# burn-research/OpenMEASURE

Measured on AMD Instinct MI355X. Metric: SPR fit+reconstruct throughput (GB/s snapshot matrix), higher is better.
Workload: dtype f64

## Files before the change

openmeasure_amd/csrc/common.hpp:

```cpp
#pragma once
#include <hip/hip_runtime.h>
#include <stdint.h>
#include <stdio.h>

#include "spr_hip.h"

typedef double f64x4 __attribute__((ext_vector_type(4)));
typedef double f64x2 __attribute__((ext_vector_type(2)));

void spr_set_error(const char *fmt, ...);

#define SPR_REQUIRE(cond, code, ...)      \
  do {                                    \
    if (!(cond)) {                        \
      spr_set_error(__VA_ARGS__);         \
      return (code);                      \
    }                                     \
  } while (0)

#define SPR_HIP_TRY(expr)                                                          \
  do {                                                                             \
    hipError_t e__ = (expr);                                                       \
    if (e__ != hipSuccess) {                                                       \
      spr_set_error("%s failed: %s (%s:%d)", #expr, hipGetErrorString(e__),       \
// ... 42 lines not shown
__host__ __device__ inline int seg_first_feature(const SegPlan &p) { return (int)(p.row0 / p.n_points); }
__host__ __device__ inline int seg_last_feature(const SegPlan &p) {
  int64_t f = (p.row0 + p.n_rows - 1) / p.n_points;
  if (f > p.n_features - 1) f = p.n_features - 1;
  return (int)f;
}

inline int seg_total_wgs(const SegPlan &p) {
  int tot = 0;
  for (int f = seg_first_feature(p); f <= seg_last_feature(p); ++f) {
    int64_t lo, hi;
    seg_range(p, f, lo, hi);
    tot += seg_wgs(p, hi - lo);
  }
  return tot;
}

__device__ inline bool seg_locate(const SegPlan &p, int b, int &f, int &wl, int &wpf, int &base,
                                  int64_t &lo, int64_t &hi) {
  int acc = 0;
  int f1 = seg_last_feature(p);
  for (int ff = seg_first_feature(p); ff <= f1; ++ff) {
    seg_range(p, ff, lo, hi);
    int w = seg_wgs(p, hi - lo);
    if (b < acc + w) {
      f = ff; wl = b - acc; wpf = w; base = acc;
      return true;
    }
    acc += w;
  }
  return false;
}

template <int CTRL>
__device__ inline double dpp_f64(double v) {
  union { double d; int i[2]; } a, b;
  a.d = v;
  b.i[0] = __builtin_amdgcn_update_dpp(0, a.i[0], CTRL, 0xF, 0xF, true);
  b.i[1] = __builtin_amdgcn_update_dpp(0, a.i[1], CTRL, 0xF, 0xF, true);
  return b.d;
}

template <int WIDTH>
__device__ inline double group_sum_t(double v) {
  if (WIDTH >= 2) v += dpp_f64<0xB1>(v);
  if (WIDTH >= 4) v += dpp_f64<0x4E>(v);
  if (WIDTH >= 8) v += dpp_f64<0x141>(v);
  if (WIDTH >= 16) v += dpp_f64<0x140>(v);
  if (WIDTH >= 32) v += __shfl_xor(v, 16, 64);
  if (WIDTH >= 64) v += __shfl_xor(v, 32, 64);
  return v;
}

__device__ inline double group_sum(double v, int width) {
  for (int o = width >> 1; o > 0; o >>= 1) v += __shfl_xor(v, o, 64);
  return v;
}

constexpr int spr_pow2_divisor_le64(int n) {
  int p = 1;
  while (p < 64 && n % (2 * p) == 0) p *= 2;
  return p;
}

inline int spr_round_mt(int m) {
  static const int sup[] = {1, 2, 3, 4, 6, 8, 12, 16};
  int need = (m + 15) / 16;
  for (int s : sup)
    if (s >= need) return s;
  return -1;
}
```

openmeasure_amd/csrc/qr_pivot.hip:

```cpp
#include <stdlib.h>

#include <type_traits>

#include "rowtile.hpp"

namespace {

constexpr int QR_THREADS = 256;
#ifndef QR_EPOCH_DEEP
#define QR_EPOCH_DEEP 0
#endif
#ifndef QR_ABLATE
#define QR_ABLATE 0
#endif
#ifndef QR_TOPT_N
#define QR_TOPT_N 16
#endif
constexpr int QR_TOPT = QR_TOPT_N;
constexpr int QR_MAX_BLOCKS = 1024;
constexpr int QR_BATCH = 16;

struct Best {
  double v1; int64_t i1; double v2;
  __device__ inline void init() { v1 = -2.0; i1 = INT64_MAX; v2 = -2.0; }
// ... 60 lines not shown
    bv = -3.0; bi = INT64_MAX; bp = -1;
    for (int e = first + lane; e < first + count; e += 64) {
      const double v = sval[e]; const long long i = sidx[e];
      if (v > bv || (v == bv && i < bi)) { bv = v; bi = i; bp = e; }
    }
    for (int o = 32; o > 0; o >>= 1) {
      const double ov = __shfl_xor(bv, o, 64);
      const long long oi = __shfl_xor(bi, o, 64);
      const int op = __shfl_xor(bp, o, 64);
      if (ov > bv || (ov == bv && oi < bi)) { bv = ov; bi = oi; bp = op; }
    }
  }
  template <int SPW>
  __device__ inline void block_merge(double *sval, long long *sidx, double *out, bool owner, int slot) {
    constexpr int NWV = QR_THREADS / 64;
    __shared__ double wv[NWV * QR_TOPT];
    __shared__ long long wi[NWV * QR_TOPT];
    const int lane = threadIdx.x & 63, wave = threadIdx.x >> 6;
    if (owner) {
#pragma unroll
      for (int k = 0; k < QR_TOPT; ++k) {
        sval[(wave * SPW + slot) * QR_TOPT + k] = tv[k];
        sidx[(wave * SPW + slot) * QR_TOPT + k] = ti[k] >= 0 ? (long long)ti[k] + base : -1;
      }
    }
    __syncthreads();
    for (int round = 0; round < QR_TOPT; ++round) {
      double bv; long long bi; int bp;
      argmax_round(sval, sidx, wave * SPW * QR_TOPT, SPW * QR_TOPT, lane, bv, bi, bp);
      if (lane == 0) {
        wv[wave * QR_TOPT + round] = bv;
        wi[wave * QR_TOPT + round] = bi;
        if (bp >= 0) sval[bp] = -3.0;
      }
      __builtin_amdgcn_wave_barrier();
    }
    __syncthreads();
    if (wave == 0) {
      for (int round = 0; round < QR_TOPT; ++round) {
        double bv; long long bi; int bp;
        argmax_round(wv, wi, 0, NWV * QR_TOPT, lane, bv, bi, bp);
        if (lane == 0) {
          out[2 * round] = bv > -2.5 ? bv : -2.0;
          out[2 * round + 1] = (double)(bv > -2.5 ? bi : -1);
          if (bp >= 0) wv[bp] = -3.0;
        }
        __builtin_amdgcn_wave_barrier();
      }
    }
  }
};
using TopList = TopListT<long long>;

template <bool INIT>
struct RowOwner {
  int off, q;
  bool own;
  __device__ inline RowOwner(int lane) {
    const int g = lane >> 4, c = lane & 15;
    if (INIT) { off = c; q = c >> 2; own = (c & 3) == g; }
    else { off = g + 4 * (c & 3); q = c & 3; own = c < 4; }
  }
  __device__ inline int slot(int lane) const { return INIT ? ((lane >> 4) * 4 + ((lane & 15) >> 2)) : ((lane >> 4) * 4 + (lane & 3)); }
  __device__ inline double pick(double v0, double v1, double v2, double v3) const {
    return q == 0 ? v0 : q == 1 ? v1 : q == 2 ? v2 : v3;
  }
};
constexpr int QR_SPW = 16;

template <int MTR, int VEC, typename TU, bool INIT>
__global__ __launch_bounds__(QR_THREADS) void qr_refresh_mfma_kernel(
    const TU *__restrict__ Ur, int64_t n_rows, int r, int64_t ldu, int64_t row0,
    const double *__restrict__ Q, int nq, double *__restrict__ nrm, double *__restrict__ tops) {
  constexpr int NW = QR_THREADS / 64, R = 64;
  constexpr int MPAD = 16 * MTR, MP = MPAD + 2, KSTEPS = MPAD / 4;
  using RT = RowTile<MTR, R, MP, NW, 16, TU>;
  constexpr int SPW = QR_SPW;
  constexpr int PANELS = 2 * R * MP, MERGE = 2 * (QR_THREADS / 64) * SPW * QR_TOPT;
  __shared__ double smem[PANELS > MERGE ? PANELS : MERGE];
  double *const lds0 = smem, *const lds1 = smem + R * MP;
  double *const sval = smem;
  long long *const sidx = reinterpret_cast<long long *>(smem + (QR_THREADS / 64) * SPW * QR_TOPT);
  const int lane = threadIdx.x & 63;
  const int wave = __builtin_amdgcn_readfirstlane(threadIdx.x >> 6);

  double bfrag[KSTEPS];
#pragma unroll
  for (int ks = 0; ks < KSTEPS; ++ks) {
    const int k = 4 * ks + (lane >> 4), j = lane & 15;
    bfrag[ks] = (!INIT && j < nq && k < r) ? Q[(int64_t)j * r + k] : 0.0;
  }
  TopList top;
  top.init();
  const RowOwner<INIT> who(lane);
  RT tile;
  const int64_t npanels = (n_rows + R - 1) / R;
  int64_t c = blockIdx.x;
  if (c < npanels) {
    tile.template load<VEC>(Ur, ldu, r, c * R, n_rows, wave, lane);
    tile.raw_store(lds0, r, c * R, n_rows, wave, lane);
    int64_t cn = c + gridDim.x;
    int64_t nrow0 = (cn < npanels) ? cn * R : n_rows;
    tile.template load<VEC>(Ur, ldu, r, nrow0, n_rows, wave, lane);
    int buf = 0;
    const int afrag = (lane & 15) * MP + (lane >> 4);
    auto old_of = [&](int64_t row0p) {
      const int64_t rr = row0p + wave * 16 + who.off;
      return (INIT || QR_ABLATE >= 2) ? 0.0 : nrm[rr < n_rows ? rr : n_rows - 1];
    };
    double old = old_of(c * R), old_n = old_of(nrow0);
    while (c < npanels) {
      const double *cur = buf ? lds1 : lds0;
      double *nxt = buf ? lds0 : lds1;
      const int64_t c2 = cn + gridDim.x;
      const int64_t n2row0 = (c2 < npanels) ? c2 * R : n_rows;
      __syncthreads();
      const int64_t orow = c * R + wave * 16 + who.off;
      const bool mine = who.own && orow < n_rows;
      const double old_n2 = old_of(n2row0);
      const double *p = cur + wave * 16 * MP + afrag;
      f64x4 acc = {0.0, 0.0, 0.0, 0.0};
#pragma unroll
      for (int ks = 0; ks < KSTEPS; ++ks) {
        const double a = p[4 * ks];
        acc = __builtin_amdgcn_mfma_f64_16x16x4f64(a, INIT ? a : bfrag[ks], acc, 0, 0, 0);
        if (ks == 0) {
#pragma unroll
          for (int it = 0; it < RT::IT; ++it) {
            tile.raw_store_pass(it, nxt, r, nrow0, n_rows, wave, lane);
            tile.template load_pass<VEC>(it, Ur, ldu, r, n2row0, n_rows, wave, lane);
          }
        }
      }
      double v;
      if (INIT) {
        v = who.pick(acc.x, acc.y, acc.z, acc.w);
      } else {
        const double d2 = who.pick(group_sum_t<16>(acc.x * acc.x), group_sum_t<16>(acc.y * acc.y),
                                   group_sum_t<16>(acc.z * acc.z), group_sum_t<16>(acc.w * acc.w));
        v = old - d2;
        v = v < 0.0 ? 0.0 : v;
        v = old < 0.0 ? -1.0 : v;
      }
      if (QR_ABLATE >= 2) asm volatile("" ::"v"(v));
      if (QR_ABLATE < 2 && mine) nrm[orow] = v;
      if (QR_ABLATE < 1) top.insert(v, row0 + orow, mine);
      old = old_n;
      old_n = old_n2;
      buf ^= 1;
      c = cn;
      cn = c2;
      nrow0 = n2row0;
    }
  }
  __syncthreads();
  top.template block_merge<SPW>(sval, sidx, tops + (int64_t)blockIdx.x * QR_TOPT * 2, who.own, who.slot(lane));
}

template <int NG, typename TU, bool INIT>
__global__ __launch_bounds__(QR_THREADS) void qr_refresh_direct_kernel(
    const TU *__restrict__ Ur, int64_t n_rows, int r, int64_t ldu, int64_t row0,
    const double *__restrict__ Q, int nq, double *__restrict__ nrm, double *__restrict__ tops) {
  constexpr int R = 64;
  constexpr int SPW = QR_SPW;
  __shared__ double smem[2 * (QR_THREADS / 64) * SPW * QR_TOPT];
  double *const sval = smem;
  long long *const sidx = reinterpret_cast<long long *>(smem + (QR_THREADS / 64) * SPW * QR_TOPT);
  const int lane = threadIdx.x & 63;
  const int wave = __builtin_amdgcn_readfirstlane(threadIdx.x >> 6);
  const int li = lane & 15, kk = lane >> 4;
  using P4 = typename std::conditional<std::is_same<TU, float>::value, float4, double4>::type;

  double bfrag[4 * NG];
#pragma unroll
  for (int g = 0; g < NG; ++g)
#pragma unroll
    for (int t = 0; t < 4; ++t)
      bfrag[4 * g + t] = (!INIT && li < nq) ? Q[(int64_t)li * r + 16 * g + 4 * kk + t] : 0.0;
  TopList top;
  top.init();
  const RowOwner<INIT> who(lane);
  const int64_t npanels = (n_rows + R - 1) / R;
  auto load_block = [&](int64_t c, P4 (&dst)[NG]) {
    int64_t row = c * R + wave * 16 + li;
    row = row < n_rows ? row : n_rows - 1;
    const TU *rp = Ur + row * ldu + 4 * kk;
#pragma unroll
    for (int g = 0; g < NG; ++g) dst[g] = *reinterpret_cast<const P4 *>(rp + 16 * g);
  };
  auto old_of = [&](int64_t cc) {
    const int64_t rr = cc * R + wave * 16 + who.off;
    return INIT ? 0.0 : nrm[rr < n_rows ? rr : n_rows - 1];
  };
  int64_t c = blockIdx.x;
  P4 cur[NG], nxt[NG];
  double old = 0.0;
  if (c < npanels) { load_block(c, cur); old = old_of(c); }
  while (c < npanels) {
    const int64_t cn = c + gridDim.x;
    load_block(cn < npanels ? cn : c, nxt);
    const double old_n = old_of(cn < npanels ? cn : c);
    const int64_t orow = c * R + wave * 16 + who.off;
    const bool mine = who.own && orow < n_rows;
    f64x4 acc = {0.0, 0.0, 0.0, 0.0};
#pragma unroll
    for (int g = 0; g < NG; ++g) {
      const double a4[4] = {(double)cur[g].x, (double)cur[g].y, (double)cur[g].z, (double)cur[g].w};
#pragma unroll
      for (int t = 0; t < 4; ++t)
        acc = __builtin_amdgcn_mfma_f64_16x16x4f64(a4[t], INIT ? a4[t] : bfrag[4 * g + t], acc, 0, 0, 0);
    }
    double v;
    if (INIT) {
      v = who.pick(acc.x, acc.y, acc.z, acc.w);
    } else {
      const double d2 = who.pick(group_sum_t<16>(acc.x * acc.x), group_sum_t<16>(acc.y * acc.y),
                                 group_sum_t<16>(acc.z * acc.z), group_sum_t<16>(acc.w * acc.w));
      v = old - d2;
      v = v < 0.0 ? 0.0 : v;
      v = old < 0.0 ? -1.0 : v;
    }
    if (mine) nrm[orow] = v;
    top.insert(v, row0 + orow, mine);
#pragma unroll
    for (int g = 0; g < NG; ++g) cur[g] = nxt[g];
    old = old_n;
    c = cn;
  }
  top.template block_merge<SPW>(sval, sidx, tops + (int64_t)blockIdx.x * QR_TOPT * 2, who.own, who.slot(lane));
}

template <int NGMAX, int VEC, typename TU, bool INIT>
__global__ __launch_bounds__(QR_THREADS) void qr_refresh_wide_kernel(
    const TU *__restrict__ Ur, int64_t n_rows, int r, int64_t ldu, int64_t row0,
    const double *__restrict__ Q, int nq, double *__restrict__ nrm, double *__restrict__ tops) {
  constexpr int R = 64, SG = 8;
  constexpr int SPW = QR_SPW;
  __shared__ double smem[2 * (QR_THREADS / 64) * SPW * QR_TOPT];
  __shared__ double Ql[INIT ? 16 : NGMAX * 256];
  double *const sval = smem;
  long long *const sidx = reinterpret_cast<long long *>(smem + (QR_THREADS / 64) * SPW * QR_TOPT);
  const int lane = threadIdx.x & 63;
  const int wave = __builtin_amdgcn_readfirstlane(threadIdx.x >> 6);
  const int li = lane & 15, kk = lane >> 4;
  const int ng = (r + 15) / 16;
  using P4 = typename std::conditional<std::is_same<TU, float>::value, float4, double4>::type;

  if (!INIT) {
    for (int e = threadIdx.x; e < ng * 256; e += QR_THREADS) {
      const int j = e & 15, k4 = (e >> 4) & 3, t = (e >> 6) & 3, g = e >> 8;
      const int k = 16 * g + 4 * k4 + t;
      Ql[e] = (j < nq && k < r) ? Q[(int64_t)j * r + k] : 0.0;
    }
    __syncthreads();
  }
  TopList top;
  top.init();
  const RowOwner<INIT> who(lane);
  const int64_t npanels = (n_rows + R - 1) / R;
  auto load_batch = [&](const TU *rp, int g0, P4 (&dst)[SG]) {
#pragma unroll
    for (int u = 0; u < SG; ++u) {
      const int g = g0 + u < ng ? g0 + u : ng - 1;
      const int c0 = 16 * g + 4 * kk;
      if (VEC) {
        dst[u] = *reinterpret_cast<const P4 *>(rp + c0);
      } else {
        dst[u].x = c0 < r ? rp[c0] : (TU)0;         dst[u].y = c0 + 1 < r ? rp[c0 + 1] : (TU)0;
        dst[u].z = c0 + 2 < r ? rp[c0 + 2] : (TU)0; dst[u].w = c0 + 3 < r ? rp[c0 + 3] : (TU)0;
      }
    }
  };
  for (int64_t c = blockIdx.x; c < npanels; c += gridDim.x) {
    int64_t row = c * R + wave * 16 + li;
    row = row < n_rows ? row : n_rows - 1;
    const TU *rp = Ur + row * ldu;
    const int64_t orow = c * R + wave * 16 + who.off;
    const bool mine = who.own && orow < n_rows;
    const double old = INIT ? 0.0 : nrm[orow < n_rows ? orow : n_rows - 1];
    f64x4 acc = {0.0, 0.0, 0.0, 0.0};
    P4 cur[SG], nxt[SG];
    load_batch(rp, 0, cur);
    for (int g0 = 0; g0 < ng; g0 += SG) {
      load_batch(rp, g0 + SG, nxt);
#pragma unroll
      for (int u = 0; u < SG; ++u) {
        if (g0 + u < ng) {
          const double a4[4] = {(double)cur[u].x, (double)cur[u].y, (double)cur[u].z, (double)cur[u].w};
          const double *ql = Ql + (int64_t)(g0 + u) * 256 + kk * 16 + li;
#pragma unroll
          for (int t = 0; t < 4; ++t)
            acc = __builtin_amdgcn_mfma_f64_16x16x4f64(a4[t], INIT ? a4[t] : ql[64 * t], acc, 0, 0, 0);
        }
      }
#pragma unroll
      for (int u = 0; u < SG; ++u) cur[u] = nxt[u];
    }
    double v;
    if (INIT) {
      v = who.pick(acc.x, acc.y, acc.z, acc.w);
    } else {
      const double d2 = who.pick(group_sum_t<16>(acc.x * acc.x), group_sum_t<16>(acc.y * acc.y),
                                 group_sum_t<16>(acc.z * acc.z), group_sum_t<16>(acc.w * acc.w));
      v = old - d2;
      v = v < 0.0 ? 0.0 : v;
      v = old < 0.0 ? -1.0 : v;
    }
    if (mine) nrm[orow] = v;
    top.insert(v, row0 + orow, mine);
  }
  top.template block_merge<SPW>(sval, sidx, tops + (int64_t)blockIdx.x * QR_TOPT * 2, who.own, who.slot(lane));
}

__global__ __launch_bounds__(QR_THREADS) void qr_tops_from_norms_kernel(const double *__restrict__ nrm0, int64_t n_rows,
                                                                        int64_t row0, double *__restrict__ nrm,
                                                                        double *__restrict__ tops) {
  constexpr int R = 64, NWV = QR_THREADS / 64, SPW = 64;
  __shared__ double smem[2 * NWV * SPW * QR_TOPT];
  double *const sval = smem;
  long long *const sidx = reinterpret_cast<long long *>(smem + NWV * SPW * QR_TOPT);
  const int lane = threadIdx.x & 63, wave = threadIdx.x >> 6;
  TopList top;
  top.init();
  const int64_t npanels = (n_rows + R - 1) / R;
  const int64_t stride = (int64_t)gridDim.x * NWV;
  int64_t c = blockIdx.x + (int64_t)wave * gridDim.x;
  for (; (c + 3 * stride + 1) * R <= n_rows; c += 4 * stride) {
    double v[4];
#pragma unroll
    for (int u = 0; u < 4; ++u) v[u] = nrm0[(c + u * stride) * R + lane];
#pragma unroll
    for (int u = 0; u < 4; ++u) {
      const int64_t row = (c + u * stride) * R + lane;
      nrm[row] = v[u];
      top.insert(v[u], row0 + row, true);
    }
  }
  for (; c < npanels; c += stride) {
    const int64_t row = c * R + lane;
    const bool mine = row < n_rows;
    const double v = nrm0[mine ? row : n_rows - 1];
    if (mine) nrm[row] = v;
    top.insert(v, row0 + row, mine);
  }
  top.template block_merge<SPW>(sval, sidx, tops + (int64_t)blockIdx.x * QR_TOPT * 2, true, lane);
}

template <typename TU>
__global__ __launch_bounds__(QR_THREADS) void qr_gather_kernel(
    const double *__restrict__ tops, const TU *__restrict__ Ur, int r, int64_t ldu, int64_t row0,
    int64_t n_rows, int ldc, int64_t *__restrict__ cand_idx, double *__restrict__ cand_res,
    double *__restrict__ cand_U) {
  const int b = blockIdx.x;
  for (int e = threadIdx.x; e < QR_TOPT * ldc; e += QR_THREADS) {
    const int k = e / ldc, c = e - k * ldc;
    const double v = tops[((int64_t)b * QR_TOPT + k) * 2];
// ... 485 lines not shown
    else if (r <= 512) RWV(32);
    else RWV(64);
#undef RWV
#undef RW
    SPR_LAUNCH_CHECK();
    return SPR_OK;
  }
  const int mtr = spr_round_mt(r);
  const int lm = vec_ok ? ((r == 16 * mtr) ? 2 : 1) : 0;
  static const bool direct_on = [] { const char *e = getenv("SPR_QR_DIRECT"); return !(e && e[0] == '0'); }();
  const bool want_direct = INIT || std::is_same<TU, float>::value;
  if (direct_on && want_direct && r % 16 == 0 && (ldu * sizeof(TU)) % 16 == 0 &&
      (reinterpret_cast<uintptr_t>(Ur) & 15) == 0) {
#define RD(NGV) hipLaunchKernelGGL((qr_refresh_direct_kernel<NGV, TU, INIT>), dim3(grid), dim3(QR_THREADS), 0, st, Ur, n_rows, r, ldu, row0, Qj, nq, nrm, tops)
    switch (r / 16) {
      case 1: RD(1); break;
      case 2: RD(2); break;
      case 3: RD(3); break;
      case 4: RD(4); break;
      case 5: RD(5); break;
      case 6: RD(6); break;
      case 7: RD(7); break;
      default: RD(8); break;
    }
#undef RD
    SPR_LAUNCH_CHECK();
    return SPR_OK;
  }
#define RF(MTV, LM) hipLaunchKernelGGL((qr_refresh_mfma_kernel<MTV, LM, TU, INIT>), dim3(grid), dim3(QR_THREADS), 0, st, Ur, n_rows, r, ldu, row0, Qj, nq, nrm, tops)
#define RFV(MTV) do { if (lm == 2) RF(MTV, 2); else if (lm == 1) RF(MTV, 1); else RF(MTV, 0); } while (0)
  switch (mtr) {
    case 1: RFV(1); break;
    case 2: RFV(2); break;
    case 3: RFV(3); break;
    case 4: RFV(4); break;
    case 6: RFV(6); break;
    default: RFV(8); break;
  }
#undef RFV
#undef RF
  SPR_LAUNCH_CHECK();
  return SPR_OK;
}

int check_ur(const char *who, const void *Ur, int64_t n_rows, int32_t r, int64_t ldu) {
  SPR_REQUIRE(Ur != nullptr, SPR_E_INVALID, "%s: Ur is NULL", who);
  SPR_REQUIRE(n_rows > 0 && r > 0 && ldu >= r, SPR_E_INVALID, "%s: bad shape n_rows=%lld r=%d ldu=%lld", who,
              (long long)n_rows, r, (long long)ldu);
  SPR_REQUIRE(r <= SPR_MAX_R_WIDE, SPR_E_UNSUPPORTED, "%s: r=%d > %d not built", who, r, SPR_MAX_R_WIDE);
  return SPR_OK;
}

template <int NG, int NTT, typename P4>
__device__ inline void epoch_tiles_mfma(const P4 (&cur)[NG], const double *__restrict__ ql0, double (&q2)[4]) {
  f64x4 acc[NTT];
#pragma unroll
  for (int tl = 0; tl < NTT; ++tl) acc[tl] = f64x4{0.0, 0.0, 0.0, 0.0};
#pragma unroll
  for (int g = 0; g < NG; ++g) {
    const double a4[4] = {(double)cur[g].x, (double)cur[g].y, (double)cur[g].z, (double)cur[g].w};
#pragma unroll
    for (int t = 0; t < 4; ++t) {
#pragma unroll
      for (int tl = 0; tl < NTT; ++tl)
        acc[tl] = __builtin_amdgcn_mfma_f64_16x16x4f64(a4[t], ql0[tl * NG * 256 + (g * 4 + t) * 64], acc[tl], 0, 0, 0);
    }
  }
#pragma unroll
  for (int tl = 0; tl < NTT; ++tl) {
    q2[0] = fma(acc[tl].x, acc[tl].x, q2[0]); q2[1] = fma(acc[tl].y, acc[tl].y, q2[1]);
    q2[2] = fma(acc[tl].z, acc[tl].z, q2[2]); q2[3] = fma(acc[tl].w, acc[tl].w, q2[3]);
  }
}

template <int NG, int NT, typename TU, bool POOL, bool ILP = false>
__global__ __launch_bounds__(QR_THREADS, (NG <= 4 && !ILP ? 3 : 2)) void qr_epoch_sweep_kernel(
    const TU *__restrict__ Ur, int64_t n_rows, int r, int64_t ldu, int64_t row0, const double *__restrict__ Q, int nq,
    double *__restrict__ nrm_e, double *__restrict__ nrm, const int32_t *__restrict__ pool,
    const int32_t *__restrict__ pool_n_ptr, double *__restrict__ tops) {
  constexpr int R = 64, SPW = QR_SPW;
  __shared__ double smem[2 * (QR_THREADS / 64) * SPW * QR_TOPT];
  __shared__ double Ql[NT * NG * 256];
  double *const sval = smem;
  long long *const sidx = reinterpret_cast<long long *>(smem + (QR_THREADS / 64) * SPW * QR_TOPT);
  const int lane = threadIdx.x & 63;
  const int wave = __builtin_amdgcn_readfirstlane(threadIdx.x >> 6);
  const int li = lane & 15, kk = lane >> 4;
  using P4 = typename std::conditional<std::is_same<TU, float>::value, float4, double4>::type;
  const int nt = (nq + 15) / 16;
  for (int e = threadIdx.x; e < nt * NG * 256; e += QR_THREADS) {
    const int j = e & 15, k4 = (e >> 4) & 3, t = (e >> 6) & 3, g = (e >> 8) % NG, tile = (e >> 8) / NG;
    const int d = 16 * tile + j;
    Ql[e] = (d < nq) ? Q[(int64_t)d * r + 16 * g + 4 * k4 + t] : 0.0;
  }
  __syncthreads();
  TopListT<int> top;
  top.init();
  top.base = row0;
  const RowOwner<false> who(lane);
  const int64_t n_units = POOL ? (int64_t)*pool_n_ptr : n_rows;
  const int64_t npanels = (n_units + R - 1) / R;
  auto slot_row = [&](int64_t c) -> int64_t {
    const int64_t u = c * R + wave * 16 + li;
    if (u >= n_units) return -1;
    return POOL ? (int64_t)pool[u] : u;
  };
  auto load_block = [&](int64_t row, P4 (&dst)[NG]) {
    const TU *rp = Ur + (row >= 0 ? row : 0) * ldu + 4 * kk;
#pragma unroll
    for (int g = 0; g < NG; ++g) dst[g] = *reinterpret_cast<const P4 *>(rp + 16 * g);
  };
  auto own_row = [&](int64_t row) -> int64_t {
    const int lo = __shfl((int)(row & 0xffffffff), who.off, 64), hi = __shfl((int)(row >> 32), who.off, 64);
    return ((int64_t)hi << 32) | (uint32_t)lo;
  };
  constexpr int NBUF = (QR_EPOCH_DEEP && NG * sizeof(P4) / 4 <= 32 && NG <= 6) ? 3 : 2;
  P4 buf[NBUF][NG];
  double oldv[NBUF];
  int64_t orv[NBUF];
  auto fetch = [&](int64_t cc, P4 (&dst)[NG], double &old, int64_t &orow) {
    const int64_t row = cc < npanels ? slot_row(cc) : -1;
    load_block(row, dst);
    orow = own_row(row);
    old = nrm_e[orow >= 0 ? orow : 0];
  };
  auto process = [&](const P4 (&cur)[NG], double old, int64_t orow) {
    const bool mine = who.own && orow >= 0;
    double q2[4] = {0.0, 0.0, 0.0, 0.0};
    if (ILP) {
      const double *ql0 = Ql + kk * 16 + li;
      if (nt == 1) epoch_tiles_mfma<NG, 1, P4>(cur, ql0, q2);
      else if (nt == 2) epoch_tiles_mfma<NG, (NT >= 2 ? 2 : 1), P4>(cur, ql0, q2);
      else if (nt == 3) epoch_tiles_mfma<NG, (NT >= 3 ? 3 : 1), P4>(cur, ql0, q2);
      else epoch_tiles_mfma<NG, (NT >= 4 ? 4 : 1), P4>(cur, ql0, q2);
    } else
    for (int tile = 0; tile < nt; ++tile) {
      const double *ql = Ql + tile * NG * 256 + kk * 16 + li;
      f64x4 acc = {0.0, 0.0, 0.0, 0.0};
#pragma unroll
      for (int g = 0; g < NG; ++g) {
        const double a4[4] = {(double)cur[g].x, (double)cur[g].y, (double)cur[g].z, (double)cur[g].w};
#pragma unroll
        for (int t = 0; t < 4; ++t)
          acc = __builtin_amdgcn_mfma_f64_16x16x4f64(a4[t], ql[(g * 4 + t) * 64], acc, 0, 0, 0);
      }
      q2[0] = fma(acc.x, acc.x, q2[0]); q2[1] = fma(acc.y, acc.y, q2[1]);
      q2[2] = fma(acc.z, acc.z, q2[2]); q2[3] = fma(acc.w, acc.w, q2[3]);
    }
    const double d2 = who.pick(group_sum_t<16>(q2[0]), group_sum_t<16>(q2[1]), group_sum_t<16>(q2[2]), group_sum_t<16>(q2[3]));
    double v = old - d2;
    v = v < 0.0 ? 0.0 : v;
    v = old < 0.0 ? -1.0 : v;
    if (mine) {
      nrm[orow] = v;
      if (!POOL) nrm_e[orow] = v;
    }
    top.insert(v, (int)orow, mine);
  };
  int64_t c = blockIdx.x;
  const int64_t gs = gridDim.x;
#pragma unroll
  for (int u = 0; u < NBUF - 1; ++u) fetch(c + u * gs, buf[u], oldv[u], orv[u]);
  while (c < npanels) {
#pragma unroll
    for (int u = 0; u < NBUF; ++u) {
      if (c < npanels) {
        constexpr int NB1 = NBUF - 1;
        fetch(c + NB1 * gs, buf[(u + NB1) % NBUF], oldv[(u + NB1) % NBUF], orv[(u + NB1) % NBUF]);
        process(buf[u], oldv[u], orv[u]);
        c += gs;
      }
    }
  }
  top.template block_merge<SPW>(sval, sidx, tops + (int64_t)blockIdx.x * QR_TOPT * 2, who.own, who.slot(lane));
}

constexpr int PB_THREADS = 256;
constexpr int PB_MAX_BLOCKS = 2048;

__global__ __launch_bounds__(PB_THREADS) void qr_pool_count_kernel(const double *__restrict__ nrm_e, int64_t n_rows,
                                                                   int64_t chunk, double theta, int32_t *__restrict__ counts) {
  __shared__ int red[PB_THREADS / 64];
  const int64_t lo = (int64_t)blockIdx.x * chunk, hi = lo + chunk < n_rows ? lo + chunk : n_rows;
  int cnt = 0;
  for (int64_t i = lo + threadIdx.x; i < hi; i += PB_THREADS) cnt += nrm_e[i] > theta;
  for (int o = 32; o > 0; o >>= 1) cnt += __shfl_xor(cnt, o, 64);
  if ((threadIdx.x & 63) == 0) red[threadIdx.x >> 6] = cnt;
  __syncthreads();
  if (threadIdx.x == 0) {
    int t = 0;
    for (int w = 0; w < PB_THREADS / 64; ++w) t += red[w];
    counts[blockIdx.x] = t;
  }
}

__global__ __launch_bounds__(1024) void qr_pool_scan_kernel(int32_t *__restrict__ counts, int n_blocks, int64_t cap,
                                                            int32_t *__restrict__ pool_n) {
  constexpr int PER = (PB_MAX_BLOCKS + 1023) / 1024;
  __shared__ int wsum[16];
  const int t = threadIdx.x, lane = t & 63, wave = t >> 6;
  int v[PER], mine = 0;
#pragma unroll
  for (int i = 0; i < PER; ++i) {
    const int b = t * PER + i;
    v[i] = b < n_blocks ? counts[b] : 0;
    mine += v[i];
  }
  int incl = mine;
  for (int o = 1; o < 64; o <<= 1) {
    const int up = __shfl_up(incl, o, 64);
    if (lane >= o) incl += up;
  }
  if (lane == 63) wsum[wave] = incl;
  __syncthreads();
  int before = 0, total = 0;
  for (int w = 0; w < 16; ++w) { if (w < wave) before += wsum[w]; total += wsum[w]; }
  int run = before + incl - mine;
#pragma unroll
  for (int i = 0; i < PER; ++i) {
    const int b = t * PER + i;
    if (b < n_blocks) counts[b] = run;
    run += v[i];
  }
  if (t == 0) *pool_n = (int64_t)total <= cap ? total : -1;
}

__global__ __launch_bounds__(PB_THREADS) void qr_pool_fill_kernel(const double *__restrict__ nrm_e, int64_t n_rows,
// ... 260 lines not shown
                                  const int64_t *d_piv, int32_t nq, double d_min, void *stream) {
  SPR_REQUIRE(d_nrm && n_rows > 0 && row0 >= 0 && n_points > 0, SPR_E_INVALID, "spr_qr_exclude_f64: bad arguments");
  SPR_REQUIRE(nq >= 0 && nq <= QR_BATCH && (nq == 0 || (d_xyz && d_piv)), SPR_E_INVALID,
              "spr_qr_exclude_f64: nq=%d picks need xyz and piv (at most %d per call)", nq, QR_BATCH);
  SPR_REQUIRE(!d_xyz || (xyz_dim >= 1 && xyz_dim <= 3), SPR_E_INVALID, "spr_qr_exclude_f64: xyz needs 1..3 columns");
  if (!d_mask && nq == 0) return SPR_OK;
  int64_t blocks = (n_rows + QR_THREADS - 1) / QR_THREADS;
  if (blocks > 4096) blocks = 4096;
  hipLaunchKernelGGL(qr_exclude_kernel, dim3((int)blocks), dim3(QR_THREADS), 0, static_cast<hipStream_t>(stream), d_nrm,
                     n_rows, row0, n_points, d_mask, d_xyz, (int)xyz_dim, d_piv, (int)nq, d_min);
  SPR_LAUNCH_CHECK();
  return SPR_OK;
}

template <typename TU>
static int qr_refresh_entry(const char *who, const TU *d_Ur, int64_t n_rows, int32_t r, int64_t ldu, int64_t row0,
                            const double *d_Q, const int64_t *d_piv, int32_t j0, int32_t nq, double *d_nrm,
                            double *d_rec, double *d_tau, void *d_workspace, size_t workspace_bytes, void *stream) {
  int rc = check_ur(who, d_Ur, n_rows, r, ldu);
  if (rc != SPR_OK) return rc;
  SPR_REQUIRE(d_Q && d_piv && d_nrm && d_rec && d_tau && d_workspace, SPR_E_INVALID, "%s: NULL pointer", who);
  SPR_REQUIRE(j0 >= 0 && nq >= 1 && nq <= QR_BATCH && j0 + nq <= r, SPR_E_INVALID, "%s: bad j0=%d nq=%d", who, j0, nq);
  SPR_REQUIRE(workspace_bytes >= QrWs::bytes(r), SPR_E_WORKSPACE, "%s: workspace too small", who);
  hipStream_t st = static_cast<hipStream_t>(stream);
  const int grid = sweep_grid(n_rows);
  const int vec_ok = (r % 2 == 0) && (ldu % 2 == 0) && ((reinterpret_cast<uintptr_t>(d_Ur) & (2 * sizeof(TU) - 1)) == 0);
  QrWs w(d_workspace, r);
  hipLaunchKernelGGL(qr_mark_kernel, dim3(1), dim3(64), 0, st, d_piv + j0, (int)nq, row0, n_rows, d_nrm);
  SPR_LAUNCH_CHECK();
  rc = launch_refresh<TU, false>(grid, st, d_Ur, n_rows, (int)r, ldu, vec_ok, row0, d_Q + (int64_t)j0 * r, (int)nq, d_nrm, w.tops);
  if (rc != SPR_OK) return rc;
  return build_candidates<TU>(w, grid, d_Ur, n_rows, r, ldu, row0, d_rec, d_tau, st);
}

extern "C" int spr_qr_refresh_f64(const double *d_Ur, int64_t n_rows, int32_t r, int64_t ldu, int64_t row0,
                                  const double *d_Q, const int64_t *d_piv, int32_t j0, int32_t nq, double *d_nrm,
                                  double *d_rec, double *d_tau, void *d_workspace, size_t workspace_bytes,
                                  void *stream) {
  return qr_refresh_entry("spr_qr_refresh_f64", d_Ur, n_rows, r, ldu, row0, d_Q, d_piv, j0, nq, d_nrm, d_rec, d_tau,
                          d_workspace, workspace_bytes, stream);
}

extern "C" int spr_qr_refresh_u32(const float *d_Ur, int64_t n_rows, int32_t r, int64_t ldu, int64_t row0,
                                  const double *d_Q, const int64_t *d_piv, int32_t j0, int32_t nq, double *d_nrm,
                                  double *d_rec, double *d_tau, void *d_workspace, size_t workspace_bytes,
                                  void *stream) {
  return qr_refresh_entry("spr_qr_refresh_u32", d_Ur, n_rows, r, ldu, row0, d_Q, d_piv, j0, nq, d_nrm, d_rec, d_tau,
                          d_workspace, workspace_bytes, stream);
}

extern "C" int32_t spr_qr_epoch_supported(int32_t r, int64_t ldu, const void *d_Ur, int32_t u_is_f32, int64_t n_rows) {
  const size_t es = u_is_f32 ? sizeof(float) : sizeof(double);
  return r >= 16 && r <= SPR_MAX_R && r % 16 == 0 && (ldu * es) % 16 == 0 && (reinterpret_cast<uintptr_t>(d_Ur) & 15) == 0 &&
         n_rows > 0 && n_rows < INT32_MAX;
}

extern "C" int32_t spr_qr_epoch_max_directions(int32_t r) {
  const int ng = r / 16;
  return 16 * (ng < 4 ? ng : ng <= 6 ? 4 : 3);
}

extern "C" size_t spr_qr_pool_workspace(void) { return sizeof(int32_t) * (PB_MAX_BLOCKS + 4); }

extern "C" int spr_qr_pool_build(const double *d_nrm_e, int64_t n_rows, double theta, int32_t *d_pool, int64_t cap,
                                 int32_t *d_pool_n, void *d_workspace, size_t workspace_bytes, void *stream) {
  SPR_REQUIRE(d_nrm_e && d_pool && d_pool_n && d_workspace, SPR_E_INVALID, "spr_qr_pool_build: NULL pointer");
  SPR_REQUIRE(n_rows > 0 && n_rows < INT32_MAX && cap > 0, SPR_E_INVALID, "spr_qr_pool_build: bad shape");
  SPR_REQUIRE(workspace_bytes >= spr_qr_pool_workspace(), SPR_E_WORKSPACE, "spr_qr_pool_build: workspace too small");
  hipStream_t st = static_cast<hipStream_t>(stream);
  int64_t chunk = (n_rows + PB_MAX_BLOCKS - 1) / PB_MAX_BLOCKS;
  chunk = (chunk + PB_THREADS - 1) / PB_THREADS * PB_THREADS;
  const int blocks = (int)((n_rows + chunk - 1) / chunk);
  int32_t *counts = static_cast<int32_t *>(d_workspace);
  hipLaunchKernelGGL(qr_pool_count_kernel, dim3(blocks), dim3(PB_THREADS), 0, st, d_nrm_e, n_rows, chunk, theta, counts);
  SPR_LAUNCH_CHECK();
  hipLaunchKernelGGL(qr_pool_scan_kernel, dim3(1), dim3(1024), 0, st, counts, blocks, cap, d_pool_n);
  SPR_LAUNCH_CHECK();
  hipLaunchKernelGGL(qr_pool_fill_kernel, dim3(blocks), dim3(PB_THREADS), 0, st, d_nrm_e, n_rows, chunk, theta, counts,
                     d_pool_n, d_pool);
  SPR_LAUNCH_CHECK();
  return SPR_OK;
}

template <typename TU>
static int qr_epoch_entry(const char *who, const TU *d_Ur, int64_t n_rows, int32_t r, int64_t ldu, int64_t row0,
                          const double *d_Q, const int64_t *d_piv, int32_t j_e, int32_t j, int32_t j_mark,
                          double *d_nrm_e, double *d_nrm, const int32_t *d_pool, const int32_t *d_pool_n,
                          int64_t pool_n_host, double tau_floor, double *d_rec, double *d_tau, void *d_workspace,
                          size_t workspace_bytes, void *stream) {
  int rc = check_ur(who, d_Ur, n_rows, r, ldu);
  if (rc != SPR_OK) return rc;
  SPR_REQUIRE(d_Q && d_piv && d_nrm_e && d_nrm && d_rec && d_tau && d_workspace, SPR_E_INVALID, "%s: NULL pointer", who);
  SPR_REQUIRE(spr_qr_epoch_supported(r, ldu, d_Ur, std::is_same<TU, float>::value, n_rows), SPR_E_UNSUPPORTED,
              "%s: r=%d / alignment outside the epoch sweep's range (r a multiple of 16 up to %d, 16-byte rows)", who, r, SPR_MAX_R);
  SPR_REQUIRE(j_e >= 0 && j > j_e && j <= r && j - j_e <= spr_qr_epoch_max_directions(r) && j_mark >= 0 && j_mark <= j,
              SPR_E_INVALID, "%s: bad direction range [%d, %d) (at most %d per sweep), marks from %d", who, j_e, j,
              spr_qr_epoch_max_directions(r), j_mark);
  SPR_REQUIRE(!d_pool || (d_pool_n && pool_n_host >= 1 && pool_n_host <= n_rows), SPR_E_INVALID, "%s: bad pool", who);
  SPR_REQUIRE(workspace_bytes >= QrWs::bytes(r), SPR_E_WORKSPACE, "%s: workspace too small", who);
  hipStream_t st = static_cast<hipStream_t>(stream);
  QrWs w(d_workspace, r);
  for (int m0 = j_mark; m0 < j; m0 += 64) {
    const int nm = j - m0 < 64 ? j - m0 : 64;
    hipLaunchKernelGGL(qr_mark_kernel, dim3(1), dim3(64), 0, st, d_piv + m0, nm, row0, n_rows, d_nrm_e);
    hipLaunchKernelGGL(qr_mark_kernel, dim3(1), dim3(64), 0, st, d_piv + m0, nm, row0, n_rows, d_nrm);
  }
  SPR_LAUNCH_CHECK();
// ... 59 lines not shown
```

Baseline: 1104.

## Transpose MFMA operands so row norms reduce via permlane swaps and wave-level top list

Swaps the A/B operands of the f64 MFMA in the refresh and epoch kernels so each row's projection lands across lanes of a column. The squared norm then reduces with two permlane16/permlane32 swaps instead of four 16-wide DPP/shuffle reductions. The epoch kernel also replaces the per-slot top-K list with a wave-level sorted list kept one entry per lane, uses 32-bit row offsets for addressing, and shrinks shared memory. It adds a stride limit on the epoch path and relies on MI355X-specific permlane swap builtins.

```diff
diff --git a/openmeasure_amd/csrc/common.hpp b/openmeasure_amd/csrc/common.hpp
--- a/openmeasure_amd/csrc/common.hpp
+++ b/openmeasure_amd/csrc/common.hpp
@@ -118,6 +118,19 @@
   return v;
 }
 
+__device__ inline double rows_sum_f64(double v) {
+  union { double d; unsigned u[2]; } a, lo, hi;
+  a.d = v;
+  const auto s0 = __builtin_amdgcn_permlane16_swap(a.u[0], a.u[0], false, false);
+  const auto s1 = __builtin_amdgcn_permlane16_swap(a.u[1], a.u[1], false, false);
+  lo.u[0] = s0[0]; lo.u[1] = s1[0]; hi.u[0] = s0[1]; hi.u[1] = s1[1];
+  a.d = lo.d + hi.d;
+  const auto t0 = __builtin_amdgcn_permlane32_swap(a.u[0], a.u[0], false, false);
+  const auto t1 = __builtin_amdgcn_permlane32_swap(a.u[1], a.u[1], false, false);
+  lo.u[0] = t0[0]; lo.u[1] = t1[0]; hi.u[0] = t0[1]; hi.u[1] = t1[1];
+  return lo.d + hi.d;
+}
+
 __device__ inline double group_sum(double v, int width) {
   for (int o = width >> 1; o > 0; o >>= 1) v += __shfl_xor(v, o, 64);
   return v;
diff --git a/openmeasure_amd/csrc/qr_pivot.hip b/openmeasure_amd/csrc/qr_pivot.hip
--- a/openmeasure_amd/csrc/qr_pivot.hip
+++ b/openmeasure_amd/csrc/qr_pivot.hip
@@ -136,20 +136,79 @@
 };
 using TopList = TopListT<long long>;
 
+template <typename TI>
+struct WaveTopT {
+  static_assert(QR_TOPT <= 16 && sizeof(TI) == 4, "one list entry per lane of a 16-lane row; 32-bit row indices");
+  double tv, thr;
+  TI ti;
+  long long base = 0;
+  bool first;
+  __device__ inline void init(int lane) { tv = -2.0; thr = -2.0; ti = -1; first = (lane & 15) == 0; }
+  __device__ static inline double bcast(double v, int l) {
+    union { double d; int i[2]; } a, b;
+    a.d = v;
+    b.i[0] = __builtin_amdgcn_readlane(a.i[0], l);
+    b.i[1] = __builtin_amdgcn_readlane(a.i[1], l);
+    return b.d;
+  }
+  __device__ inline void insert(double v, TI gi, bool mine) {
+    unsigned long long m = __ballot(mine && v > thr);
+    while (m) {
+      const int l = __builtin_ctzll(m);
+      m &= m - 1;
+      const double cv = bcast(v, l);
+      const TI ci = (TI)__builtin_amdgcn_readlane((int)gi, l);
+      if (cv > thr) {
+        const double upv = dpp_f64<0x111>(tv);
+        const TI upi = (TI)__builtin_amdgcn_update_dpp(0, (int)ti, 0x111, 0xF, 0xF, true);
+        const bool stay = tv >= cv, here = first || upv >= cv;
+        ti = stay ? ti : (here ? ci : upi);
+        tv = stay ? tv : (here ? cv : upv);
+        thr = bcast(tv, QR_TOPT - 1);
+      }
+    }
+  }
+  __device__ inline void block_merge(double *wv, long long *wi, double *out) {
+    constexpr int NWV = QR_THREADS / 64;
+    const int lane = threadIdx.x & 63, wave = threadIdx.x >> 6;
+    if (lane < QR_TOPT) {
+      wv[wave * QR_TOPT + lane] = tv;
+      wi[wave * QR_TOPT + lane] = ti >= 0 ? (long long)ti + base : -1;
+    }
+    __syncthreads();
+    if (wave == 0) {
+      for (int round = 0; round < QR_TOPT; ++round) {
+        double bv; long long bi; int bp;
+        TopList::argmax_round(wv, wi, 0, NWV * QR_TOPT, lane, bv, bi, bp);
+        if (lane == 0) {
+          out[2 * round] = bv > -2.5 ? bv : -2.0;
+          out[2 * round + 1] = (double)(bv > -2.5 ? bi : -1);
+          if (bp >= 0) wv[bp] = -3.0;
+        }
+        __builtin_amdgcn_wave_barrier();
+      }
+    }
+  }
+};
+
 template <bool INIT>
 struct RowOwner {
   int off, q;
   bool own;
   __device__ inline RowOwner(int lane) {
     const int g = lane >> 4, c = lane & 15;
-    if (INIT) { off = c; q = c >> 2; own = (c & 3) == g; }
-    else { off = g + 4 * (c & 3); q = c & 3; own = c < 4; }
-  }
-  __device__ inline int slot(int lane) const { return INIT ? ((lane >> 4) * 4 + ((lane & 15) >> 2)) : ((lane >> 4) * 4 + (lane & 3)); }
+    off = c;
+    q = c >> 2;
+    own = INIT ? (c & 3) == g : g == 0;
+  }
+  __device__ inline int slot(int lane) const { return INIT ? ((lane >> 4) * 4 + ((lane & 15) >> 2)) : (lane & 15); }
   __device__ inline double pick(double v0, double v1, double v2, double v3) const {
     return q == 0 ? v0 : q == 1 ? v1 : q == 2 ? v2 : v3;
   }
 };
+__device__ inline double tile_sq_sum(f64x4 acc) {
+  return rows_sum_f64(fma(acc.x, acc.x, acc.y * acc.y) + fma(acc.z, acc.z, acc.w * acc.w));
+}
 constexpr int QR_SPW = 16;
 
 template <int MTR, int VEC, typename TU, bool INIT>
@@ -207,7 +266,8 @@
 #pragma unroll
       for (int ks = 0; ks < KSTEPS; ++ks) {
         const double a = p[4 * ks];
-        acc = __builtin_amdgcn_mfma_f64_16x16x4f64(a, INIT ? a : bfrag[ks], acc, 0, 0, 0);
+        acc = INIT ? __builtin_amdgcn_mfma_f64_16x16x4f64(a, a, acc, 0, 0, 0)
+                   : __builtin_amdgcn_mfma_f64_16x16x4f64(bfrag[ks], a, acc, 0, 0, 0);
         if (ks == 0) {
 #pragma unroll
           for (int it = 0; it < RT::IT; ++it) {
@@ -220,8 +280,7 @@
       if (INIT) {
         v = who.pick(acc.x, acc.y, acc.z, acc.w);
       } else {
-        const double d2 = who.pick(group_sum_t<16>(acc.x * acc.x), group_sum_t<16>(acc.y * acc.y),
-                                   group_sum_t<16>(acc.z * acc.z), group_sum_t<16>(acc.w * acc.w));
+        const double d2 = tile_sq_sum(acc);
         v = old - d2;
         v = v < 0.0 ? 0.0 : v;
         v = old < 0.0 ? -1.0 : v;
@@ -292,14 +351,14 @@
       const double a4[4] = {(double)cur[g].x, (double)cur[g].y, (double)cur[g].z, (double)cur[g].w};
 #pragma unroll
       for (int t = 0; t < 4; ++t)
-        acc = __builtin_amdgcn_mfma_f64_16x16x4f64(a4[t], INIT ? a4[t] : bfrag[4 * g + t], acc, 0, 0, 0);
+        acc = INIT ? __builtin_amdgcn_mfma_f64_16x16x4f64(a4[t], a4[t], acc, 0, 0, 0)
+                   : __builtin_amdgcn_mfma_f64_16x16x4f64(bfrag[4 * g + t], a4[t], acc, 0, 0, 0);
     }
     double v;
     if (INIT) {
       v = who.pick(acc.x, acc.y, acc.z, acc.w);
     } else {
-      const double d2 = who.pick(group_sum_t<16>(acc.x * acc.x), group_sum_t<16>(acc.y * acc.y),
-                                 group_sum_t<16>(acc.z * acc.z), group_sum_t<16>(acc.w * acc.w));
+      const double d2 = tile_sq_sum(acc);
       v = old - d2;
       v = v < 0.0 ? 0.0 : v;
       v = old < 0.0 ? -1.0 : v;
@@ -374,7 +433,8 @@
           const double *ql = Ql + (int64_t)(g0 + u) * 256 + kk * 16 + li;
 #pragma unroll
           for (int t = 0; t < 4; ++t)
-            acc = __builtin_amdgcn_mfma_f64_16x16x4f64(a4[t], INIT ? a4[t] : ql[64 * t], acc, 0, 0, 0);
+            acc = INIT ? __builtin_amdgcn_mfma_f64_16x16x4f64(a4[t], a4[t], acc, 0, 0, 0)
+                       : __builtin_amdgcn_mfma_f64_16x16x4f64(ql[64 * t], a4[t], acc, 0, 0, 0);
         }
       }
 #pragma unroll
@@ -384,8 +444,7 @@
     if (INIT) {
       v = who.pick(acc.x, acc.y, acc.z, acc.w);
     } else {
-      const double d2 = who.pick(group_sum_t<16>(acc.x * acc.x), group_sum_t<16>(acc.y * acc.y),
-                                 group_sum_t<16>(acc.z * acc.z), group_sum_t<16>(acc.w * acc.w));
+      const double d2 = tile_sq_sum(acc);
       v = old - d2;
       v = v < 0.0 ? 0.0 : v;
       v = old < 0.0 ? -1.0 : v;
@@ -977,7 +1036,7 @@
 }
 
 template <int NG, int NTT, typename P4>
-__device__ inline void epoch_tiles_mfma(const P4 (&cur)[NG], const double *__restrict__ ql0, double (&q2)[4]) {
+__device__ inline double epoch_tiles_mfma(const P4 (&cur)[NG], const double *__restrict__ ql0) {
   f64x4 acc[NTT];
 #pragma unroll
   for (int tl = 0; tl < NTT; ++tl) acc[tl] = f64x4{0.0, 0.0, 0.0, 0.0};
@@ -988,14 +1047,16 @@
     for (int t = 0; t < 4; ++t) {
 #pragma unroll
       for (int tl = 0; tl < NTT; ++tl)
-        acc[tl] = __builtin_amdgcn_mfma_f64_16x16x4f64(a4[t], ql0[tl * NG * 256 + (g * 4 + t) * 64], acc[tl], 0, 0, 0);
-    }
-  }
+        acc[tl] = __builtin_amdgcn_mfma_f64_16x16x4f64(ql0[tl * NG * 256 + (g * 4 + t) * 64], a4[t], acc[tl], 0, 0, 0);
+    }
+  }
+  double s0 = 0.0, s1 = 0.0;
 #pragma unroll
   for (int tl = 0; tl < NTT; ++tl) {
-    q2[0] = fma(acc[tl].x, acc[tl].x, q2[0]); q2[1] = fma(acc[tl].y, acc[tl].y, q2[1]);
-    q2[2] = fma(acc[tl].z, acc[tl].z, q2[2]); q2[3] = fma(acc[tl].w, acc[tl].w, q2[3]);
-  }
+    s0 = fma(acc[tl].x, acc[tl].x, s0); s1 = fma(acc[tl].y, acc[tl].y, s1);
+    s0 = fma(acc[tl].z, acc[tl].z, s0); s1 = fma(acc[tl].w, acc[tl].w, s1);
+  }
+  return s0 + s1;
 }
 
 template <int NG, int NT, typename TU, bool POOL, bool ILP = false>
@@ -1003,11 +1064,10 @@
     const TU *__restrict__ Ur, int64_t n_rows, int r, int64_t ldu, int64_t row0, const double *__restrict__ Q, int nq,
     double *__restrict__ nrm_e, double *__restrict__ nrm, const int32_t *__restrict__ pool,
     const int32_t *__restrict__ pool_n_ptr, double *__restrict__ tops) {
-  constexpr int R = 64, SPW = QR_SPW;
-  __shared__ double smem[2 * (QR_THREADS / 64) * SPW * QR_TOPT];
+  constexpr int R = 64;
+  __shared__ double wv[(QR_THREADS / 64) * QR_TOPT];
+  __shared__ long long wi[(QR_THREADS / 64) * QR_TOPT];
   __shared__ double Ql[NT * NG * 256];
-  double *const sval = smem;
-  long long *const sidx = reinterpret_cast<long long *>(smem + (QR_THREADS / 64) * SPW * QR_TOPT);
   const int lane = threadIdx.x & 63;
   const int wave = __builtin_amdgcn_readfirstlane(threadIdx.x >> 6);
   const int li = lane & 15, kk = lane >> 4;
@@ -1019,60 +1079,69 @@
     Ql[e] = (d < nq) ? Q[(int64_t)d * r + 16 * g + 4 * k4 + t] : 0.0;
   }
   __syncthreads();
-  TopListT<int> top;
-  top.init();
+  WaveTopT<int> top;
+  top.init(lane);
   top.base = row0;
-  const RowOwner<false> who(lane);
+  const bool owner = kk == 0;
   const int64_t n_units = POOL ? (int64_t)*pool_n_ptr : n_rows;
   const int64_t npanels = (n_units + R - 1) / R;
-  auto slot_row = [&](int64_t c) -> int64_t {
-    const int64_t u = c * R + wave * 16 + li;
-    if (u >= n_units) return -1;
-    return POOL ? (int64_t)pool[u] : u;
-  };
-  auto load_block = [&](int64_t row, P4 (&dst)[NG]) {
-    const TU *rp = Ur + (row >= 0 ? row : 0) * ldu + 4 * kk;
-#pragma unroll
-    for (int g = 0; g < NG; ++g) dst[g] = *reinterpret_cast<const P4 *>(rp + 16 * g);
-  };
-  auto own_row = [&](int64_t row) -> int64_t {
-    const int lo = __shfl((int)(row & 0xffffffff), who.off, 64), hi = __shfl((int)(row >> 32), who.off, 64);
-    return ((int64_t)hi << 32) | (uint32_t)lo;
-  };
+  const int slot = wave * 16 + li;
+  const uint32_t ldub = (uint32_t)(ldu * sizeof(TU));
+  const uint32_t kkb = (uint32_t)(4 * kk * sizeof(TU));
   constexpr int NBUF = (QR_EPOCH_DEEP && NG * sizeof(P4) / 4 <= 32 && NG <= 6) ? 3 : 2;
   P4 buf[NBUF][NG];
   double oldv[NBUF];
-  int64_t orv[NBUF];
-  auto fetch = [&](int64_t cc, P4 (&dst)[NG], double &old, int64_t &orow) {
-    const int64_t row = cc < npanels ? slot_row(cc) : -1;
-    load_block(row, dst);
-    orow = own_row(row);
-    old = nrm_e[orow >= 0 ? orow : 0];
+  int orv[NBUF];
+  auto fetch = [&](int64_t cc, P4 (&dst)[NG], double &old, int &orow) {
+    const bool live = cc < npanels;
+    if (POOL) {
+      const int64_t u = cc * R + slot;
+      orow = (live && u < n_units) ? pool[u] : -1;
+      const int64_t row = orow >= 0 ? orow : 0;
+      const TU *rp = Ur + row * ldu + 4 * kk;
+#pragma unroll
+      for (int g = 0; g < NG; ++g) dst[g] = *reinterpret_cast<const P4 *>(rp + 16 * g);
+      old = nrm_e[row];
+    } else {
+      const int64_t base = live ? cc * R : 0;
+      const int64_t rest = n_units - base;
+      const int left = live ? (int)(rest < R ? rest : R) : 1;
+      const int rl = slot < left ? slot : left - 1;
+      const char *ub = reinterpret_cast<const char *>(Ur + base * ldu);
+      const uint32_t off = (uint32_t)rl * ldub + kkb;
+#pragma unroll
+      for (int g = 0; g < NG; ++g) dst[g] = *reinterpret_cast<const P4 *>(ub + off + (uint32_t)(16 * g * sizeof(TU)));
+      old = (nrm_e + base)[rl];
+      orow = (live && slot < left) ? (int)base + slot : -1;
+    }
   };
-  auto process = [&](const P4 (&cur)[NG], double old, int64_t orow) {
-    const bool mine = who.own && orow >= 0;
-    double q2[4] = {0.0, 0.0, 0.0, 0.0};
+  auto process = [&](const P4 (&cur)[NG], double old, int orow) {
+    const bool mine = owner && orow >= 0;
+    double q2;
     if (ILP) {
       const double *ql0 = Ql + kk * 16 + li;
-      if (nt == 1) epoch_tiles_mfma<NG, 1, P4>(cur, ql0, q2);
-      else if (nt == 2) epoch_tiles_mfma<NG, (NT >= 2 ? 2 : 1), P4>(cur, ql0, q2);
-      else if (nt == 3) epoch_tiles_mfma<NG, (NT >= 3 ? 3 : 1), P4>(cur, ql0, q2);
-      else epoch_tiles_mfma<NG, (NT >= 4 ? 4 : 1), P4>(cur, ql0, q2);
-    } else
-    for (int tile = 0; tile < nt; ++tile) {
-      const double *ql = Ql + tile * NG * 256 + kk * 16 + li;
-      f64x4 acc = {0.0, 0.0, 0.0, 0.0};
-#pragma unroll
-      for (int g = 0; g < NG; ++g) {
-        const double a4[4] = {(double)cur[g].x, (double)cur[g].y, (double)cur[g].z, (double)cur[g].w};
-#pragma unroll
-        for (int t = 0; t < 4; ++t)
-          acc = __builtin_amdgcn_mfma_f64_16x16x4f64(a4[t], ql[(g * 4 + t) * 64], acc, 0, 0, 0);
+      if (nt == 1) q2 = epoch_tiles_mfma<NG, 1, P4>(cur, ql0);
+      else if (nt == 2) q2 = epoch_tiles_mfma<NG, (NT >= 2 ? 2 : 1), P4>(cur, ql0);
+      else if (nt == 3) q2 = epoch_tiles_mfma<NG, (NT >= 3 ? 3 : 1), P4>(cur, ql0);
+      else q2 = epoch_tiles_mfma<NG, (NT >= 4 ? 4 : 1), P4>(cur, ql0);
+    } else {
+      double s0 = 0.0, s1 = 0.0;
+      for (int tile = 0; tile < nt; ++tile) {
+        const double *ql = Ql + tile * NG * 256 + kk * 16 + li;
+        f64x4 acc = {0.0, 0.0, 0.0, 0.0};
+#pragma unroll
+        for (int g = 0; g < NG; ++g) {
+          const double a4[4] = {(double)cur[g].x, (double)cur[g].y, (double)cur[g].z, (double)cur[g].w};
+#pragma unroll
+          for (int t = 0; t < 4; ++t)
+            acc = __builtin_amdgcn_mfma_f64_16x16x4f64(ql[(g * 4 + t) * 64], a4[t], acc, 0, 0, 0);
+        }
+        s0 = fma(acc.x, acc.x, s0); s1 = fma(acc.y, acc.y, s1);
+        s0 = fma(acc.z, acc.z, s0); s1 = fma(acc.w, acc.w, s1);
       }
-      q2[0] = fma(acc.x, acc.x, q2[0]); q2[1] = fma(acc.y, acc.y, q2[1]);
-      q2[2] = fma(acc.z, acc.z, q2[2]); q2[3] = fma(acc.w, acc.w, q2[3]);
-    }
-    const double d2 = who.pick(group_sum_t<16>(q2[0]), group_sum_t<16>(q2[1]), group_sum_t<16>(q2[2]), group_sum_t<16>(q2[3]));
+      q2 = s0 + s1;
+    }
+    const double d2 = rows_sum_f64(q2);
     double v = old - d2;
     v = v < 0.0 ? 0.0 : v;
     v = old < 0.0 ? -1.0 : v;
@@ -1080,7 +1149,7 @@
       nrm[orow] = v;
       if (!POOL) nrm_e[orow] = v;
     }
-    top.insert(v, (int)orow, mine);
+    top.insert(v, orow, mine);
   };
   int64_t c = blockIdx.x;
   const int64_t gs = gridDim.x;
@@ -1097,7 +1166,7 @@
       }
     }
   }
-  top.template block_merge<SPW>(sval, sidx, tops + (int64_t)blockIdx.x * QR_TOPT * 2, who.own, who.slot(lane));
+  top.block_merge(wv, wi, tops + (int64_t)blockIdx.x * QR_TOPT * 2);
 }
 
 constexpr int PB_THREADS = 256;
@@ -1464,7 +1533,7 @@
 extern "C" int32_t spr_qr_epoch_supported(int32_t r, int64_t ldu, const void *d_Ur, int32_t u_is_f32, int64_t n_rows) {
   const size_t es = u_is_f32 ? sizeof(float) : sizeof(double);
   return r >= 16 && r <= SPR_MAX_R && r % 16 == 0 && (ldu * es) % 16 == 0 && (reinterpret_cast<uintptr_t>(d_Ur) & 15) == 0 &&
-         n_rows > 0 && n_rows < INT32_MAX;
+         n_rows > 0 && n_rows < INT32_MAX && ldu * (int64_t)es < (1 << 25);
 }
 
 extern "C" int32_t spr_qr_epoch_max_directions(int32_t r) {
```

Measured after the change: 1104, median of 2. Within noise of the previous version (+0.0%).
